# td-kwj-zp2023/webgpu-msm-twisted-edwards

Measured on AMD Instinct MI355X. Metric: MSMs/sec at n=2^20 Twisted-Edwards BLS12 (pipelined throughput = 1000/ms_per_step; single-MSM latency in latency_ms), higher is better.
Workload: dtype u32

## Files before the change

webgpu-msm-twisted-edwards_amd/csrc/kernels.hip.hpp:

```cpp
#pragma once
#include <hip/hip_runtime.h>
#include "curve.hpp"

namespace te {

#define TE_BATCH_MAX 8
struct batch_ptrs { const uint4* p[TE_BATCH_MAX]; };
struct batch_slabs { uint32_t s[TE_BATCH_MAX]; };

struct digits_params {
  uint32_t half[10];
  uint32_t zero_digit;
  uint32_t sc_stride;
  uint32_t n, nst;
  int num_windows;
  int w_first, w_step, nw_local;
  uint32_t half_code, logS, P, CH, chunk_len;
};

struct pnt_slot { uint4 q[8]; };
__device__ __forceinline__ void prep_points_block(uint32_t blk, uint4* __restrict__ lds, const uint4* __restrict__ pts, pnt_slot* __restrict__ recs, uint32_t n) {
  const uint32_t t = threadIdx.x, base = blk * 256u;
  const bool active = t < 256u;
  const uint32_t pieces_in = (n - base < 256u ? n - base : 256u) * 4u;
  const uint4* __restrict__ src = pts + (size_t)base * 4u;
  if (active) {
#pragma unroll
    for (int j = 0; j < 4; j++) {
      const uint32_t g = (uint32_t)j * 256u + t;
      lds[g] = src[g < pieces_in ? g : 0u];
    }
  }
  __syncthreads();
  uint4 a0 = make_uint4(0u, 0u, 0u, 0u), a1 = a0, b0 = a0, b1 = a0;
  if (active) { a0 = lds[4 * t + 0]; a1 = lds[4 * t + 1]; b0 = lds[4 * t + 2]; b1 = lds[4 * t + 3]; }
// ... 519 lines not shown
  __syncthreads();
  const uint32_t c0 = cnt_s[t];
  const size_t gb = (size_t)k * g.B + (size_t)p * g.S + t;
  if (!single) {
    if (c0) atomicAdd(&a.bucket_count[gb], c0);
    wait_own_accesses();
    __syncthreads();
    if (t == 0) pj[2] = (handoff_arrive(&a.part_ticket[k * g.P + p]) + 1u == (cntp + TE_L2_CAP - 1u) / TE_L2_CAP) ? 1u : 0u;
    __syncthreads();
    if (pj[2]) (void)seg_plan_block(p, k, t < g.S ? ld_agent(a.bucket_count + gb) : 0u, g, a.pa, PL, pb, cntp, sbp);
    return;
  }
  if (t < g.S) a.bucket_count[gb] = c0;
  const uint32_t ex = seg_plan_block(p, k, c0, g, a.pa, PL, pb, cntp, sbp);
  if (t < g.S) a.pa.bucket_cursor[gb] = pb + ex + c0;
  off_s[t] = ex;
  __syncthreads();
#pragma unroll
  for (int c = 0; c < 5; c++) {
    uint32_t kv[8], iv[8]; piece_group<PK>(r, c, kv, iv);
    const uint32_t e0 = ((uint32_t)c * 256u + t) * 8u;
#pragma unroll
    for (int e = 0; e < 8; e++) {
      const uint32_t pos = e0 + (uint32_t)e;
      if (pos >= head && pos < total) list[atomicAdd(&off_s[kv[e] & 0x7fffu], 1u)] = iv[e] | ((kv[e] >> 15) << 31);
    }
  }
  __syncthreads();
  uint32_t* out = a.sorted + (size_t)k * g.n + pb;
  for (uint32_t s = t; s < cntp; s += 256u) out[s] = list[s];
}

#define TE_ORDER_REGS 32u
__device__ __forceinline__ void order_scatter_block(uint32_t ob, uint32_t nob, uint32_t* __restrict__ lds, const uint32_t* __restrict__ lenv, uint32_t ids,
                                                    const uint32_t* __restrict__ size_hist, uint32_t* __restrict__ rel_cursor,
                                                    uint32_t* __restrict__ order, uint32_t* __restrict__ num_segments, uint32_t max_len) {
  uint32_t* const h = lds; uint32_t* const base = lds + 1024; uint32_t* const sm = lds + 2048;
  const uint32_t per = (ids + nob - 1) / nob;
  const uint32_t lo = min(ids, ob * per), hi = min(ids, lo + per);
  const bool in_regs = per <= TE_ORDER_REGS * 256u;
  uint32_t lv[TE_ORDER_REGS];
  if (in_regs) {
#pragma unroll
    for (uint32_t j = 0; j < TE_ORDER_REGS; j++) { const uint32_t g = lo + j * 256u + threadIdx.x; lv[j] = g < hi ? lenv[g] : TE_SEG_INVALID; }
  }
  for (uint32_t j = threadIdx.x; j < 1024u; j += 256u) h[j] = 0;
  {
    uint32_t run = 0;
    for (uint32_t c = (1023u - min(max_len, 1023u)) >> 8; c < 4u; c++) {
      const uint32_t s = 1023u - (c * 256u + threadIdx.x);
      uint32_t part[TE_HIST_COPIES];
#pragma unroll
      for (uint32_t r = 0; r < TE_HIST_COPIES; r++) part[r] = size_hist[r * 1024u + s];
      uint32_t cnt_s = 0;
#pragma unroll
      for (uint32_t r = 0; r < TE_HIST_COPIES; r++) cnt_s += part[r];
      uint32_t bt;
      const uint32_t ex = block_excl_scan(cnt_s, sm, bt);
      base[s] = run + ex;
      run += bt;
    }
    if (ob == 0 && threadIdx.x == 0) *num_segments = run;
  }
  __syncthreads();
  if (in_regs) {
#pragma unroll
    for (uint32_t j = 0; j < TE_ORDER_REGS; j++) if (lv[j] != TE_SEG_INVALID) atomicAdd(&h[min(lv[j], 1023u)], 1u);
  } else {
    for (uint32_t g = lo + threadIdx.x; g < hi; g += 256u) { const uint32_t l = lenv[g]; if (l != TE_SEG_INVALID) atomicAdd(&h[min(l, 1023u)], 1u); }
  }
  __syncthreads();
  for (uint32_t j = threadIdx.x; j < 1024u; j += 256u) { base[j] += h[j] ? atomicAdd(&rel_cursor[j], h[j]) : 0u; h[j] = 0; }
  __syncthreads();
  if (in_regs) {
#pragma unroll
    for (uint32_t j = 0; j < TE_ORDER_REGS; j++) {
      if (lv[j] == TE_SEG_INVALID) continue;
      const uint32_t sz = min(lv[j], 1023u);
      order[base[sz] + atomicAdd(&h[sz], 1u)] = lo + j * 256u + threadIdx.x;
    }
  } else {
    for (uint32_t g = lo + threadIdx.x; g < hi; g += 256u) {
      const uint32_t l = lenv[g];
      if (l == TE_SEG_INVALID) continue;
      const uint32_t sz = min(l, 1023u);
      order[base[sz] + atomicAdd(&h[sz], 1u)] = g;
    }
  }
}

#define TE_PLACE_LDS_WORDS (4u * 256u + TE_L2_LIST + TE_L2_LIST / 4u + 2u + 17u)
template <bool PK>
__device__ __forceinline__ void l2_place_piece(uint32_t p, uint32_t k, uint32_t a0, uint32_t b0, uint32_t* __restrict__ lds,
                                               const uint16_t* __restrict__ part_keys, const uint32_t* __restrict__ part_idx,
                                               uint32_t* __restrict__ bucket_cursor, uint32_t* __restrict__ sorted, const sort_geom& g) {
  uint32_t* const cnt_s = lds; uint32_t* const lex_s = lds + 256; uint32_t* const off_s = lds + 512; uint32_t* const gbase_s = lds + 768;
  uint32_t* const list = lds + 1024;
  uint8_t* const list_b = reinterpret_cast<uint8_t*>(list + TE_L2_LIST);
  uint32_t* const sm = list + TE_L2_LIST + TE_L2_LIST / 4u + 2u;
  const uint32_t t = threadIdx.x, len = b0 - a0;
  const uint16_t* keys_row = part_keys + (size_t)k * g.nst; const uint32_t* idx_row = part_idx + (size_t)k * g.nst;
  uint32_t* out = sorted + (size_t)k * g.n;
  cnt_s[t] = 0u;
  __syncthreads();
  piece_regs r; uint32_t head, total;
  load_piece<PK>(keys_row, idx_row, a0, b0, t, true, r, head, total);
#pragma unroll
  for (int c = 0; c < 5; c++) {
    uint32_t kv[8], iv[8]; piece_group<PK>(r, c, kv, iv);
    const uint32_t e0 = ((uint32_t)c * 256u + t) * 8u;
#pragma unroll
    for (int e = 0; e < 8; e++) { const uint32_t pos = e0 + (uint32_t)e; if (pos >= head && pos < total) atomicAdd(&cnt_s[kv[e] & 0x7fffu], 1u); }
  }
  __syncthreads();
  wave0_excl_scan(cnt_s, lex_s, 256u, &sm[16]);
  {
    const uint32_t c0 = cnt_s[t];
    gbase_s[t] = c0 ? atomicAdd(&bucket_cursor[(size_t)k * g.B + (size_t)p * g.S + t], c0) : 0u;
  }
  __syncthreads();
  off_s[t] = lex_s[t];
  gbase_s[t] -= lex_s[t];
  __syncthreads();
#pragma unroll
  for (int c = 0; c < 5; c++) {
    uint32_t kv[8], iv[8]; piece_group<PK>(r, c, kv, iv);
    const uint32_t e0 = ((uint32_t)c * 256u + t) * 8u;
#pragma unroll
    for (int e = 0; e < 8; e++) {
      const uint32_t pos = e0 + (uint32_t)e;
      if (pos >= head && pos < total) {
        const uint32_t b = kv[e] & 0x7fffu;
        const uint32_t slot = atomicAdd(&off_s[b], 1u);
        list[slot] = iv[e] | ((kv[e] >> 15) << 31); list_b[slot] = (uint8_t)b;
      }
    }
  }
  __syncthreads();
  for (uint32_t s = t; s < len; s += 256u) out[gbase_s[list_b[s]] + s] = list[s];
}

struct order_args { const uint32_t* lenv; uint32_t ids; const uint32_t* size_hist; uint32_t* rel_cursor; uint32_t* order; uint32_t* num_segments; uint32_t order_cols, max_len; };
template <bool PK>
__global__ void __launch_bounds__(256, TE_L2_WAVES) k_l2_place_order(const uint16_t* __restrict__ part_keys, const uint32_t* __restrict__ part_idx,
                                                           const uint32_t* __restrict__ part_start, const uint32_t* __restrict__ part_count,
                                                           uint32_t* __restrict__ bucket_cursor, uint32_t* __restrict__ sorted, sort_geom g, order_args oa) {
  __shared__ uint32_t lds[TE_PLACE_LDS_WORDS];
  if (blockIdx.x < oa.order_cols) {
    order_scatter_block(blockIdx.y * oa.order_cols + blockIdx.x, gridDim.y * oa.order_cols, lds, oa.lenv, oa.ids, oa.size_hist, oa.rel_cursor, oa.order, oa.num_segments, oa.max_len);
    return;
  }
  const uint32_t k = gridDim.y - 1u - blockIdx.y;
  const uint32_t px = blockIdx.x - oa.order_cols, extra = gridDim.x - oa.order_cols - g.P, bx = px < extra ? g.P + px : px - extra;
  const uint32_t* pc = part_count + k * g.P;
  uint32_t p, j;
  if (!l2_piece_of_block(bx, pc, g.P, bx < g.P ? 0u : part_count[gridDim.y * g.P + k], lds, lds + 32, p, j)) return;
  const uint32_t cntp = pc[p], pb = part_start[k * g.P + p];
  if (cntp <= TE_L2_CAP) return;
  const uint32_t a0 = pb + j * TE_L2_CAP;
  l2_place_piece<PK>(p, k, a0, min(pb + cntp, a0 + TE_L2_CAP), lds, part_keys, part_idx, bucket_cursor, sorted, g);
}

template <int N> struct geo {
  static constexpr uint32_t PW = 4u * N;
  static constexpr uint32_t PQ = PW / 4u;
  static constexpr uint32_t RW = N == 9 ? 27u : 4u * N;
  static constexpr uint32_t SQ = N == 9 ? 8u : N;
  static constexpr uint32_t LQ = (RW + 3u) / 4u;
};
template <int N> struct rec_slot { uint4 q[geo<N>::SQ]; };
static_assert(sizeof(rec_slot<9>) == sizeof(pnt_slot) && sizeof(rec_slot<14>) == 224, "record slots");

template <int N> __device__ __forceinline__ pnt_t<N> load_pnt(const rec_slot<N>* __restrict__ recs, uint32_t entry) {
  const uint4* q = recs[entry & 0x7fffffffu].q;
  constexpr uint32_t LQ = geo<N>::LQ;
  uint4 u[LQ];
#pragma unroll
  for (uint32_t j = 0; j < LQ; j++) u[j] = q[j];
  uint32_t w[4 * LQ];
#pragma unroll
  for (uint32_t j = 0; j < LQ; j++) { w[4 * j] = u[j].x; w[4 * j + 1] = u[j].y; w[4 * j + 2] = u[j].z; w[4 * j + 3] = u[j].w; }
  pnt_t<N> r;
// ... 45 lines not shown
  const uint32_t* base = recs[entry & 0x7fffffffu].w;
  u4a8 u[10];
#pragma unroll
  for (int j = 0; j < 10; j++) u[j] = reinterpret_cast<const u4a8*>(base)[j];
  const u2a8 t = *reinterpret_cast<const u2a8*>(base + 40);
  uint32_t w[42];
#pragma unroll
  for (int j = 0; j < 10; j++) { w[4 * j] = u[j].v[0]; w[4 * j + 1] = u[j].v[1]; w[4 * j + 2] = u[j].v[2]; w[4 * j + 3] = u[j].v[3]; }
  w[40] = t.v[0]; w[41] = t.v[1];
  pnt_aff377 r;
#pragma unroll
  for (int j = 0; j < 14; j++) { r.hm.v[j] = w[j]; r.hp.v[j] = w[14 + j]; r.dt.v[j] = w[28 + j]; }
  return r;
}
__device__ __forceinline__ void store_pnt_aff377(rec_aff377* dst, const pnt_aff377& r) {
#pragma unroll
  for (int j = 0; j < 14; j++) { dst->w[j] = r.hm.v[j]; dst->w[14 + j] = r.hp.v[j]; dst->w[28 + j] = r.dt.v[j]; }
}
template <int N, int RK> struct rec_kind;
template <int N> struct rec_kind<N, 0> {
  using slot = rec_slot<N>; using pnt = pnt_t<N>;
  static __device__ __forceinline__ pnt load(const slot* __restrict__ recs, uint32_t e) { return load_pnt<N>(recs, e); }
};
template <> struct rec_kind<14, 1> {
  using slot = rec_aff377; using pnt = pnt_aff377;
  static __device__ __forceinline__ pnt load(const slot* __restrict__ recs, uint32_t e) { return load_pnt_aff377(recs, e); }
};

struct __attribute__((aligned(4))) idx4 { uint32_t v[4]; };
#define TE_CLK_SLOTS 64u
#define TE_IDX_STRIP 16u
template <int N, int RK = 0>
__global__ void __attribute__((amdgpu_flat_work_group_size(1, 256), amdgpu_waves_per_eu(N == 9 ? 3 : 2, N == 9 ? 3 : 2))) k_accumulate(const typename rec_kind<N, RK>::slot* __restrict__ recs, const uint32_t* __restrict__ sorted,
                                                    const uint32_t* __restrict__ bucket_start, const uint32_t* __restrict__ bucket_count,
                                                    const uint32_t* __restrict__ seg_base, const uint32_t* __restrict__ seg_bucket,
                                                    const uint32_t* __restrict__ seg_lenv, const uint32_t* __restrict__ order,
                                                    const uint32_t* __restrict__ num_segments, ete_t<N>* __restrict__ buckets,
                                                    ete_t<N>* __restrict__ seg_out, uint32_t n, uint32_t logB, uint32_t seg_len, uint32_t ids, uint32_t onto,
                                                    uint32_t win_per_msm, batch_slabs slabs, unsigned long long* __restrict__ clk) {
  __shared__ __attribute__((aligned(16))) uint32_t idx_strip[256 * TE_IDX_STRIP];
  using RT = rec_kind<N, RK>; using P = typename RT::pnt;
  unsigned long long* const slot = clk ? clk + (blockIdx.x & (TE_CLK_SLOTS - 1u)) : nullptr;
  const unsigned long long t0_wall = clk ? (unsigned long long)wall_clock64() : 0ull, t0_core = clk ? (unsigned long long)clock64() : 0ull;
  if (clk && threadIdx.x == 0) atomicMax(slot, ~t0_wall);
  const uint32_t gid = blockIdx.x * 256u + threadIdx.x;
  if (gid >= (order ? *num_segments : ids)) return;
  const uint32_t sgm = order ? order[gid] : gid;
  const uint32_t g = seg_bucket[sgm];
  if (g == TE_SEG_INVALID) return;
  const uint32_t k = g >> logB;
  recs += (size_t)slabs.s[k / win_per_msm] * n;
  const uint32_t part = sgm - seg_base[g];
  const uint32_t cnt = seg_lenv[sgm];
  const uint32_t* lst = sorted + (size_t)k * n + bucket_start[g] + part * seg_len;
  ete_t<N> acc = (onto && part == 0u) ? load_ete<N>(buckets + g) : ete_identity_t<N>();
  if (cnt) {
    const uint32_t last = cnt - 1u;
    uint32_t j0 = 0;
    uint32_t e = lst[0], e_n = lst[min(1u, last)];
    const uint32_t e_2 = lst[min(2u, last)], e_3 = lst[min(3u, last)];
    P cur = RT::load(recs, e);
    if (!(onto && part == 0u)) {
      const P first = pnt_cneg(cur, (e >> 31) != 0u);
      if (cnt >= 2u) {
        const P second = pnt_cneg(RT::load(recs, e_n), (e_n >> 31) != 0u);
        e = e_2; e_n = e_3;
        cur = RT::load(recs, e);
        acc = ete_from_pair(first, second);
        j0 = 2;
      } else {
        acc = ete_from_pnt(first);
        j0 = 1;
      }
    }
    uint32_t* const strip = idx_strip + threadIdx.x * TE_IDX_STRIP;
    auto refill = [&](uint32_t pos) {
      const idx4* src = reinterpret_cast<const idx4*>(lst + pos);
      idx4* dst = reinterpret_cast<idx4*>(strip);
#pragma unroll
      for (uint32_t h = 0; h < TE_IDX_STRIP / 4u; h += 2u) {
        const idx4 v0 = src[h], v1 = src[h + 1u];
        dst[h] = v0; dst[h + 1u] = v1;
      }
    };
    if (((j0 + 2u) & (TE_IDX_STRIP - 1u)) != 0u) refill((j0 + 2u) & ~(TE_IDX_STRIP - 1u));
    P rec_b;
    uint32_t j = j0;
    for (; j + 2u < cnt; j += 2u) {
      const uint32_t pn = j + 2u;
      if ((pn & (TE_IDX_STRIP - 1u)) == 0u) refill(pn);
      const uint2 e_nn = *reinterpret_cast<const uint2*>(strip + (pn & (TE_IDX_STRIP - 1u)));
      rec_b = RT::load(recs, e_n);
      acc = ete_madd(acc, pnt_cneg(cur, (e >> 31) != 0u));
      __builtin_amdgcn_sched_barrier(0);
      cur = RT::load(recs, e_nn.x);
      acc = ete_madd(acc, pnt_cneg(rec_b, (e_n >> 31) != 0u));
      e = e_nn.x; e_n = e_nn.y;
    }
    if (j < cnt) {
      const bool two = j + 1u < cnt;
      rec_b = RT::load(recs, two ? e_n : e);
      acc = ete_madd(acc, pnt_cneg(cur, (e >> 31) != 0u));
      if (two) acc = ete_madd(acc, pnt_cneg(rec_b, (e_n >> 31) != 0u));
    }
  }
  const bool whole = bucket_count[g] <= seg_len;
  store_ete<N>(whole ? buckets + g : seg_out + sgm, acc);
  if (clk && (uint32_t)__lane_id() == (uint32_t)__ffsll((long long)__ballot(1)) - 1u) {
    const unsigned long long t1_wall = (unsigned long long)wall_clock64(), t1_core = (unsigned long long)clock64();
    atomicMax(slot + TE_CLK_SLOTS, t1_wall);
    atomicAdd(slot + 2u * TE_CLK_SLOTS, t1_core - t0_core); atomicAdd(slot + 3u * TE_CLK_SLOTS, t1_wall - t0_wall);
  }
}

template <int N> struct sum_job_t {
  const ete_t<N>* in; ete_t<N>* out;
  uint32_t n_out;
  uint32_t K, inner;
  uint32_t in_per_window, out_per_window;
};
template <int N> struct sum_jobs_t { sum_job_t<N> j[4]; };
template <int N> __device__ __forceinline__ ete_t<N> pair_swap(const ete_t<N>& a) {
  ete_t<N> r;
#pragma unroll
  for (int i = 0; i < N; i++) {
    r.x.v[i] = (uint32_t)__builtin_amdgcn_mov_dpp((int)a.x.v[i], 0xb1, 0xf, 0xf, true);
    r.y.v[i] = (uint32_t)__builtin_amdgcn_mov_dpp((int)a.y.v[i], 0xb1, 0xf, 0xf, true);
    r.z.v[i] = (uint32_t)__builtin_amdgcn_mov_dpp((int)a.z.v[i], 0xb1, 0xf, 0xf, true);
    r.t.v[i] = (uint32_t)__builtin_amdgcn_mov_dpp((int)a.t.v[i], 0xb1, 0xf, 0xf, true);
  }
  return r;
}
template <int N, bool PAIR>
__global__ void __launch_bounds__(256, N == 9 ? 2 : 1) k_sum_groups(sum_jobs_t<N> js, uint32_t nw) {
  const sum_job_t<N>& j = js.j[blockIdx.y];
  constexpr uint32_t TPO = PAIR ? 2u : 1u;
  const uint32_t total = j.n_out * nw * TPO, Kt = j.K / TPO;
  for (uint32_t gt = blockIdx.x * 256u + threadIdx.x; gt < total; gt += gridDim.x * 256u) {
    const uint32_t g = gt / TPO, half = gt % TPO;
    const uint32_t k = g / j.n_out, o = g - k * j.n_out;
// ... 511 lines not shown
```

webgpu-msm-twisted-edwards_amd/csrc/te_msm.hip:

```cpp
#include <hip/hip_runtime.h>
#include <stdint.h>
#include <stdio.h>
#include <stdlib.h>
#include <string.h>
#include <string>
#include <vector>
#include <deque>
#include <algorithm>
#include <functional>
#include <chrono>
#include <thread>
#include <mutex>
#include <condition_variable>
#include <memory>
#include <optional>
#include <type_traits>
#if defined(__x86_64__)
#include <immintrin.h>
#endif

#include "../../include/te_msm.h"
#include "host_tail.hpp"
#include "synth.hpp"
#include "kernels.hip.hpp"
// ... 24 lines not shown
constexpr size_t TE_MAX_ROW_BYTES = TE377_TAIL_ROW_BYTES;

struct plan_t {
  int curve = 0;
  int c = 0, W = 0, nw = 0;
  int nw1 = 0, batch = 1;
  int w_first = 0, w_step = 1;
  uint32_t B = 0, logB = 0;
  int signed_digits = 1;
  uint32_t dw[4] = {0, 0, 0, 0};
  uint32_t CH = 0, chunk_len = 0, nst = 0;
  uint32_t seg_len = 64;
  uint32_t S = 0, logS = 0, P = 0;
  uint32_t packed = 0;
  int rec_kind = 0;
  int fb_rb = 0, fb_c = 0, fb_W = 0;
};

template <typename T> struct dev_buf {
  T* p = nullptr; size_t cap = 0;
  operator T*() const { return p; }
  void release() { if (p) (void)hipFree(p); p = nullptr; cap = 0; }
};

struct workset_t {
  hipStream_t stream = nullptr, copy_stream = nullptr;
  int hw_queue_class = -1;
  hipEvent_t ev_copy = nullptr, ev_start = nullptr;
  dev_buf<uint8_t> d_recs;
  dev_buf<uint16_t> d_digits, d_part_keys;
  dev_buf<uint32_t> d_part_start, d_part_count, d_part_idx, d_seg_part_base;
  dev_buf<uint32_t> d_bucket_start, d_bucket_cursor, d_sorted;
  dev_buf<uint32_t> d_seg_base, d_seg_bucket, d_seg_lenv, d_order;
  dev_buf<uint32_t> d_split_list, d_chunk_list;
  dev_buf<uint8_t> d_seg_out, d_buckets, d_red[4];
  dev_buf<uint32_t> d_zero; size_t zero_words = 0;
  size_t zero_clean_words = 0;
  uint32_t *d_err = nullptr, *d_num_seg = nullptr, *d_size_hist = nullptr, *d_size_cursor = nullptr, *d_counts1 = nullptr, *d_bucket_count = nullptr;
  uint32_t* d_part_ticket = nullptr;
  uint8_t* d_partials = nullptr;
  uint32_t* h_err = nullptr;
  uint8_t* h_partials = nullptr;
  uint32_t* h_err_dev = nullptr;
  bool rows_on_host = false;
  hipEvent_t ev_done = nullptr;
  hipEvent_t ev_result = nullptr;
  hipEvent_t ev[ST_COUNT + 1] = {};
  plan_t plan; uint64_t n = 0; bool used = false;
  te_sched::slot_t slot;
  std::string job_err;
  int prof_level = 0;
  hipStream_t last_stream = nullptr;
  dev_buf<uint8_t> d_in_points, d_in_scalars;
  std::vector<hipEvent_t> piece_events;
  uint8_t* h_ring = nullptr; std::vector<hipEvent_t> ring_ev; size_t ring_next = 0;
  uint64_t idle_calls = 0;
  dev_buf<uint32_t> d_fb_remap;
  uint32_t* d_fb_fill = nullptr;
  const void* fb_scalars = nullptr; uint64_t fb_n = 0;
  int slab = -1;
  bool slab_run = false;
  const uint8_t* recs_last = nullptr;
  te_bases* bound = nullptr;
  int pt_rc = 0; int64_t pt_index = -1; int pt_reason = 0;
  dev_buf<uint8_t> d_batch_rows;
  dev_buf<uint32_t> d_in_idx;
  template <typename WS, typename F> static void each_buffer(WS& ws, F&& f) {
    f(ws.d_recs); f(ws.d_digits); f(ws.d_part_keys); f(ws.d_part_start); f(ws.d_part_count); f(ws.d_part_idx); f(ws.d_seg_part_base);
    f(ws.d_bucket_start); f(ws.d_bucket_cursor); f(ws.d_sorted); f(ws.d_seg_base); f(ws.d_seg_bucket); f(ws.d_seg_lenv); f(ws.d_order);
    f(ws.d_split_list); f(ws.d_chunk_list); f(ws.d_seg_out); f(ws.d_buckets); for (auto& b : ws.d_red) f(b);
    f(ws.d_zero); f(ws.d_in_points); f(ws.d_in_scalars); f(ws.d_fb_remap); f(ws.d_batch_rows); f(ws.d_in_idx);
  }
};
constexpr int TE_MAX_WINDOWS = 64;
constexpr size_t Z_KEEP = 4;
constexpr size_t Z_ENTRIES = 2;
constexpr size_t Z_CLOCK = 8;
static_assert(Z_KEEP + 4 <= Z_CLOCK && Z_ENTRIES % 2 == 0 && Z_ENTRIES + 2 <= Z_KEEP, "flag words");
constexpr size_t Z_ROWS = Z_CLOCK + 4 * 2 * TE_CLK_SLOTS, Z_HIST = Z_ROWS + (size_t)TE_MAX_WINDOWS * TE_MAX_ROW_BYTES / 4, Z_CURSOR = Z_HIST + 1024 * TE_HIST_COPIES, Z_END = Z_CURSOR + 1024;

struct gpu_t {
  int device = 0;
  int w_first = 0, w_step = 1;
  workset_t ws[TE_MSM_WORKSETS];
  int last_ws = 0;
  int wall_clock_khz = 0;
  int in_flight = 0;
  bool queues_probed = false;
  struct rec_slab_t { const void* src = nullptr; uint64_t n = 0; int curve = 0; uint8_t* d = nullptr; size_t cap = 0; int users = 0;
                      uint32_t pending = 0; hipEvent_t ev[TE_MSM_WORKSETS] = {};
                      int run_users = 0; bool converted = false; hipEvent_t conv_ev = nullptr; };
  std::vector<rec_slab_t> slabs;
  std::unique_ptr<std::mutex> scalar_link{new std::mutex};
  std::unique_ptr<std::mutex> chk_mu{new std::mutex};
  hipStream_t chk_stream = nullptr; dev_buf<uint8_t> chk_pts;
  unsigned long long *chk_word = nullptr, *chk_host = nullptr;
  bool streams_exported = false;
  bool streams_final = false;
  uint8_t* h_batch_rows = nullptr; size_t h_batch_cap = 0;
};

}
// ... 144 lines not shown
}

struct seq_sizes {
  size_t wb, smax;
  size_t chunk_cap(size_t slack = 0) const { return wb + (smax + slack) / TE_GIANT_RUN + 2; }
};
inline seq_sizes sizes_for(const plan_t& p, uint64_t n) {
  const size_t wb = (size_t)p.nw * p.B;
  return {wb, wb + (size_t)p.nw * (size_t)(n / (uint64_t)p.seg_len)};
}

int ensure_buffers(te_ctx* ctx, gpu_t& d, workset_t& ws, uint64_t n, const plan_t& p, bool need_recs = true) {
  HIP_TRY(ctx, hipSetDevice(d.device));
  const seq_sizes sz = sizes_for(p, n);
  const size_t nd = (size_t)p.nw * p.nst + 64, wb = sz.wb, ab = sizes_of(p.curve).acc;
  int rc = 0;
  if (need_recs && (rc = make_room(ctx, ws.d_recs, (size_t)n * sizes_of(p.curve).rec * (size_t)p.batch))) return rc;
  if ((rc = make_room(ctx, ws.d_digits, nd))) return rc;
  if ((rc = make_room(ctx, ws.d_sorted, nd))) return rc;
  {
    const size_t c1 = (size_t)p.nw * p.CH * p.P;
    ws.zero_words = Z_END + c1 + wb + (size_t)p.nw * p.P + 64;
    { const uint32_t* before = ws.d_zero; if ((rc = make_room(ctx, ws.d_zero, ws.zero_words))) return rc; if (ws.d_zero != before) ws.zero_clean_words = 0; }
    ws.d_err = ws.d_zero; ws.d_num_seg = ws.d_zero + Z_KEEP; ws.d_size_hist = ws.d_zero + Z_HIST; ws.d_size_cursor = ws.d_zero + Z_CURSOR;
    ws.d_partials = reinterpret_cast<uint8_t*>(ws.d_zero + Z_ROWS);
    ws.d_counts1 = ws.d_zero + Z_END; ws.d_bucket_count = ws.d_counts1 + c1; ws.d_part_ticket = ws.d_bucket_count + wb;
    ws.d_fb_fill = ws.d_part_ticket + (size_t)p.nw * p.P;
  }
  if (p.fb_rb && (rc = make_room(ctx, ws.d_fb_remap, nd))) return rc;
  if ((rc = make_room(ctx, ws.d_bucket_start, wb))) return rc;
  if ((rc = make_room(ctx, ws.d_bucket_cursor, wb))) return rc;
  if ((rc = make_room(ctx, ws.d_seg_part_base, (size_t)p.nw * p.P))) return rc;
  const size_t smax = sz.smax + 16;
  if ((rc = make_room(ctx, ws.d_order, smax))) return rc;
  if ((rc = make_room(ctx, ws.d_seg_bucket, smax))) return rc;
  if ((rc = make_room(ctx, ws.d_seg_lenv, smax))) return rc;
  if ((rc = make_room(ctx, ws.d_seg_out, smax * ab))) return rc;
  if ((rc = make_room(ctx, ws.d_seg_base, wb + 1))) return rc;
  if ((rc = make_room(ctx, ws.d_split_list, wb + 1))) return rc;
  if ((rc = make_room(ctx, ws.d_chunk_list, 2 * sz.chunk_cap(16)))) return rc;
  if ((rc = make_room(ctx, ws.d_part_start, (size_t)p.nw * p.P))) return rc;
  if ((rc = make_room(ctx, ws.d_buckets, wb * ab))) return rc;
  if ((rc = make_room(ctx, ws.d_part_count, (size_t)p.nw * p.P + (size_t)p.nw))) return rc;
  if ((rc = make_room(ctx, ws.d_part_keys, p.packed ? 8 : nd))) return rc;
  if ((rc = make_room(ctx, ws.d_part_idx, nd))) return rc;
  for (int k = 0; k < 4; k++) if ((rc = make_room(ctx, ws.d_red[k], (wb / (k % 2 ? 4 : 2) + 1) * ab))) return rc;
  return 0;
}

template <int LO, int HI, typename F> void with_window_bits(int c, F&& f) {
  if constexpr (LO < HI) { if (c != LO) return with_window_bits<LO + 1, HI>(c, f); }
  f(std::integral_constant<int, LO>{});
}

template <int C> void launch_digits(const te::batch_ptrs& sc, int batch, uint16_t* dg, const te::digits_params& prm, uint32_t* err, uint32_t* counts1, hipStream_t s) {
  hipLaunchKernelGGL(te::k_digits<C>, dim3((prm.nst + TE_DIG_BLOCK - 1u) / TE_DIG_BLOCK, batch), dim3(TE_DIG_THREADS), 0, s, sc, dg, prm, err, counts1);
}
static_assert(TE_BATCH_MAX == TE_MSM_MAX_BATCH, "batch tables");
template <int C> void launch_digits_ragged(const void* sc, const te::ragged_tab& tab, int batch, uint16_t* dg, const te::digits_params& prm, uint32_t* err, uint32_t* counts1, hipStream_t s) {
  hipLaunchKernelGGL(te::k_digits_ragged<C>, dim3((prm.nst + TE_DIG_BLOCK - 1u) / TE_DIG_BLOCK, batch), dim3(TE_DIG_THREADS), 0, s, static_cast<const uint4*>(sc), tab, dg, prm, err, counts1);
}
static_assert(TE_RAGGED_MAX == TE_BATCH_SEQ_MAX && TE_BATCH_SEQ_MAX == TE_MSM_BATCH_SEQ_MAX, "ragged tables");

struct msm_launch {
  te_ctx* ctx; workset_t& ws; plan_t p;
  const void* d_points = nullptr; const void* d_scalars = nullptr; uint64_t n = 0;
  void* d_partials_out = nullptr;
// ... 95 lines not shown
          const uint32_t per_row = (n32 + 511u) / 512u;
          hipLaunchKernelGGL(te::k_part_scatter_prep377, dim3(sblocks + rows * per_row), dim3(512), 0, stream, sa, sblocks, tab, row_slab,
                             reinterpret_cast<te::rec_slot<14>*>(recs_out()), n32, per_row, rows * per_row);
        } else {
          const uint32_t per_row = (n32 + 255u) / 256u;
          hipLaunchKernelGGL(te::k_part_scatter_prep, dim3(sblocks + rows * per_row), dim3(512), 0, stream, sa, sblocks, tab, row_slab,
                             reinterpret_cast<te::pnt_slot*>(recs_out()), n32, per_row, rows * per_row);
        }
      } else if (idx) {
        hipLaunchKernelGGL(te::k_part_scatter_indexed, dim3(p.CH, p.nw), dim3(512), 0, stream, sa, te::index_args{idx, idx_count, idx_pos, ws.d_err});
      } else {
        hipLaunchKernelGGL(te::k_part_scatter, dim3(p.CH, p.nw), dim3(512), 0, stream, sa);
      }
    }
    mark(ST_BSORT);
    if (p.nw > 0) {
      const uint32_t l2_blocks = p.P + n32 / TE_L2_CAP + 1u;
      te::l2_args la;
      la.part_keys = ws.d_part_keys; la.part_idx = ws.d_part_idx; la.part_start = ws.d_part_start; la.part_count = ws.d_part_count;
      la.bucket_count = ws.d_bucket_count; la.sorted = ws.d_sorted; la.part_ticket = ws.d_part_ticket; la.g = sg;
      la.pa.part_start = ws.d_part_start; la.pa.part_count = ws.d_part_count; la.pa.seg_part_base = ws.d_seg_part_base;
      la.pa.bucket_start = ws.d_bucket_start; la.pa.bucket_cursor = ws.d_bucket_cursor; la.pa.seg_base = ws.d_seg_base; la.pa.seg_bucket = ws.d_seg_bucket;
      la.pa.seg_lenv = ws.d_seg_lenv; la.pa.size_hist = ws.d_size_hist; la.pa.split_list = ws.d_split_list; la.pa.split_count = ws.d_num_seg + 1;
      la.pa.chunk_list = ws.d_chunk_list; la.pa.seg_len = p.seg_len; la.pa.cap_w = cap_w; la.pa.chunk_cap = chunk_cap();
      if (p.packed) hipLaunchKernelGGL(te::k_l2_local<true>, dim3(l2_blocks, p.nw), dim3(256), 0, stream, la);
      else hipLaunchKernelGGL(te::k_l2_local<false>, dim3(l2_blocks, p.nw), dim3(256), 0, stream, la);
      te::order_args oa;
      oa.lenv = ws.d_seg_lenv; oa.ids = smax(); oa.size_hist = ws.d_size_hist; oa.rel_cursor = ws.d_size_cursor; oa.order = ws.d_order; oa.num_segments = ws.d_num_seg;
      {
        const uint32_t by_regs = (smax() + TE_ORDER_REGS * 256u * (uint32_t)p.nw - 1u) / (TE_ORDER_REGS * 256u * (uint32_t)p.nw);
        oa.order_cols = std::min(64u, std::max(by_regs, (uint32_t)std::max(1, 128 / p.nw)));
      }
      oa.max_len = std::min(p.seg_len, 1023u);
      if (p.packed)
        hipLaunchKernelGGL(te::k_l2_place_order<true>, dim3(oa.order_cols + l2_blocks, p.nw), dim3(256), 0, stream, ws.d_part_keys, ws.d_part_idx, ws.d_part_start,
                           ws.d_part_count, ws.d_bucket_cursor, ws.d_sorted, sg, oa);
      else
        hipLaunchKernelGGL(te::k_l2_place_order<false>, dim3(oa.order_cols + l2_blocks, p.nw), dim3(256), 0, stream, ws.d_part_keys, ws.d_part_idx, ws.d_part_start,
                           ws.d_part_count, ws.d_bucket_cursor, ws.d_sorted, sg, oa);
    }
    mark(ST_ORDER);
    return 0;
  }

  bool bls() const { return p.curve == TE_MSM_CURVE_BLS12_377_G1; }

  template <int N, int RK> int accumulate_t() {
    mark(ST_ACCUM);
    if (p.nw > 0) {
      const uint32_t n32 = this->n32(), smax = this->smax();
      const uint32_t* order = ctx->opt_sort ? ws.d_order : nullptr;
      using slot_t = typename te::rec_kind<N, RK>::slot;
      hipLaunchKernelGGL((te::k_accumulate<N, RK>), dim3((smax + 255) / 256), dim3(256), 0, stream, reinterpret_cast<const slot_t*>(bound ? bound : recs_out()), ws.d_sorted,
                         ws.d_bucket_start, ws.d_bucket_count, ws.d_seg_base, ws.d_seg_bucket, ws.d_seg_lenv, order, ws.d_num_seg,
                         reinterpret_cast<te::ete_t<N>*>(ws.d_buckets.p), reinterpret_cast<te::ete_t<N>*>(ws.d_seg_out.p), n32, p.logB, p.seg_len, smax, onto ? 1u : 0u,
                         ragged ? (uint32_t)p.nw : (uint32_t)p.nw1, ragged ? te::batch_slabs{} : slabs(),
                         prof ? reinterpret_cast<unsigned long long*>(ws.d_zero + Z_CLOCK) : nullptr);
    }
    return 0;
  }
  int accumulate() { return bls() ? (p.rec_kind == 1 ? accumulate_t<14, 1>() : accumulate_t<14, 0>()) : accumulate_t<9, 0>(); }

  template <int N> int combine_t() {
    if (p.nw <= 0) return 0;
    using E = te::ete_t<N>;
    hipLaunchKernelGGL(te::k_seg_combine_all<N>, dim3(256 + 1024), dim3(256), 0, stream, ws.d_split_list, ws.d_num_seg + 1, ws.d_chunk_list,
                       ws.d_bucket_count, ws.d_seg_base, reinterpret_cast<E*>(ws.d_seg_out.p), reinterpret_cast<E*>(ws.d_buckets.p), p.seg_len, chunk_cap(), 256u,
                       ws.d_bucket_start, ws.d_bucket_cursor);
    return 0;
  }
  int combine() { return bls() ? combine_t<14>() : combine_t<9>(); }

  template <int N> int reduce_t() {
    if (p.nw > 0) {
      using E = te::ete_t<N>;
      const uint32_t w0 = p.dw[0], w1 = p.dw[1], w2 = p.dw[2], w3 = p.dw[3];
      const uint32_t L = 1u << (w0 + w1), H = 1u << (w2 + w3);
      struct chain_t { const E* cur; uint32_t n, r; E* buf[2]; int pp; };
      E* const bk = reinterpret_cast<E*>(ws.d_buckets.p);
      chain_t ch[2] = {{bk, p.B, L, {reinterpret_cast<E*>(ws.d_red[0].p), reinterpret_cast<E*>(ws.d_red[1].p)}, 0},
                       {bk, p.B, H, {reinterpret_cast<E*>(ws.d_red[2].p), reinterpret_cast<E*>(ws.d_red[3].p)}, 0}};
      for (;;) {
        te::sum_jobs_t<N> js; memset(&js, 0, sizeof js);
        uint32_t most = 0; int nj = 0;
        for (int i = 0; i < 2; i++) {
          chain_t& c = ch[i];
          if (c.r <= 4u) continue;
          const uint32_t K = (c.r % 8u == 0) ? 8u : (c.r % 4u == 0) ? 4u : 2u;
// ... 2580 lines not shown
  if (device_index < 0 || (size_t)device_index >= ctx->devs.size() || first > total || count > total - first) return set_err(ctx, TE_MSM_EINVAL, "bad arguments");
  if (record_bytes) *record_bytes = (int)bases->rec_bytes;
  uint64_t bytes = count * bases->rec_bytes;
  if (bytes > cap) bytes = cap;
  if (!bytes) return 0;
  HIP_TRY(ctx, hipSetDevice(ctx->devs[(size_t)device_index].device));
  HIP_TRY(ctx, hipMemcpy(dst, bases->recs[(size_t)device_index] + first * bases->rec_bytes, bytes, hipMemcpyDeviceToHost));
  return (int64_t)bytes;
}

int64_t te_msm_debug_read(te_ctx* ctx, const char* stage, void* dst, uint64_t cap) {
  device_guard restore_callers_device;
  if (!ctx || !stage || !dst) return TE_MSM_EINVAL;
  drain_workers(ctx);
  gpu_t& d = ctx->devs[0];
  workset_t& ws = d.ws[d.last_ws];
  if (!ws.used) return set_err(ctx, TE_MSM_ESTATE, "no run yet");
  const plan_t& p = ws.plan; const uint64_t n = ws.n;
  const void* src = nullptr; uint64_t bytes = 0;
  if (ws.zero_clean_words && (!strcmp(stage, "bucket_count") || !strcmp(stage, "num_segments") || !strcmp(stage, "partials")))
    return set_err(ctx, TE_MSM_ESTATE, "this stage lives in the block that is cleared behind an MSM's read-back: set option prezero = 0 before the run to keep it");
  if (!strcmp(stage, "records")) {
    if (!ws.recs_last) return set_err(ctx, TE_MSM_ESTATE, "the last run gathered from a bound point set: the work set holds no records of its own");
    src = ws.recs_last; bytes = n * sizes_of(p.curve).rec;
  }
  else if (!strcmp(stage, "digits")) { src = ws.d_digits; bytes = (uint64_t)p.nw * p.nst * 2; }
  else if (!strcmp(stage, "bucket_count")) { src = ws.d_bucket_count; bytes = (uint64_t)p.nw * p.B * 4; }
  else if (!strcmp(stage, "bucket_start")) { src = ws.d_bucket_start; bytes = (uint64_t)p.nw * p.B * 4; }
  else if (!strcmp(stage, "sorted")) { src = ws.d_sorted; bytes = (uint64_t)p.nw * n * 4; }
  else if (!strcmp(stage, "num_segments")) { src = ws.d_num_seg; bytes = 4; }
  else if (!strcmp(stage, "seg_bucket")) { src = ws.d_seg_bucket; bytes = ((uint64_t)p.nw * p.B + (uint64_t)p.nw * (n / p.seg_len)) * 4; }
  else if (!strcmp(stage, "seg_len")) { src = ws.d_seg_lenv; bytes = ((uint64_t)p.nw * p.B + (uint64_t)p.nw * (n / p.seg_len)) * 4; }
  else if (!strcmp(stage, "order")) { src = ws.d_order; bytes = ((uint64_t)p.nw * p.B + (uint64_t)p.nw * (n / p.seg_len)) * 4; }
  else if (!strcmp(stage, "part_start")) { src = ws.d_part_start; bytes = (uint64_t)p.nw * p.P * 4; }
  else if (!strcmp(stage, "part_count")) { src = ws.d_part_count; bytes = (uint64_t)p.nw * p.P * 4; }
  else if (!strcmp(stage, "part_keys") && !p.packed) { src = ws.d_part_keys; bytes = (uint64_t)p.nw * p.nst * 2; }
  else if (!strcmp(stage, "part_idx") && !p.packed) { src = ws.d_part_idx; bytes = (uint64_t)p.nw * p.nst * 4; }
  else if (!strcmp(stage, "part_keys") || !strcmp(stage, "part_idx")) {
    const bool want_keys = stage[5] == 'k';
    const uint64_t words = (uint64_t)p.nw * p.nst;
    std::vector<uint32_t> pk(words);
    HIP_TRY(ctx, hipSetDevice(d.device));
    HIP_TRY(ctx, hipDeviceSynchronize());
    HIP_TRY(ctx, hipMemcpy(pk.data(), ws.d_part_idx, words * 4, hipMemcpyDeviceToHost));
    uint64_t out_bytes = words * (want_keys ? 2 : 4);
    if (out_bytes > cap) out_bytes = cap;
    if (want_keys) { uint16_t* o = static_cast<uint16_t*>(dst); for (uint64_t i = 0; i < out_bytes / 2; i++) o[i] = (uint16_t)(((pk[i] >> 23) & 0xffu) | ((pk[i] >> 31) << 15)); }
    else { uint32_t* o = static_cast<uint32_t*>(dst); for (uint64_t i = 0; i < out_bytes / 4; i++) o[i] = pk[i] & 0x7fffffu; }
    return (int64_t)out_bytes;
  }
  else if (!strcmp(stage, "buckets")) { src = ws.d_buckets; bytes = (uint64_t)p.nw * p.B * sizes_of(p.curve).acc; }
  else if (!strcmp(stage, "partials")) { src = ws.d_partials; bytes = (uint64_t)p.W * sizes_of(p.curve).row; }
  else return set_err(ctx, TE_MSM_EINVAL, "unknown stage");
  if (bytes > cap) bytes = cap;
  HIP_TRY(ctx, hipSetDevice(d.device));
  HIP_TRY(ctx, hipDeviceSynchronize());
  HIP_TRY(ctx, hipMemcpy(dst, src, bytes, hipMemcpyDeviceToHost));
  return (int64_t)bytes;
}

}
```

Baseline: 1148.

## Precompute packed segment descriptors in order scatter for accumulate kernel

The order-scatter stage now writes a 16-byte descriptor per segment, either in sorted order or indexed by id. It packs bucket, list position, count, id and first/whole flags. The accumulate kernel reads this one coalesced uint4 instead of chasing order, seg_bucket, seg_base, bucket_start, bucket_count and seg_lenv through dependent gathers. This removes the latency of the indirect-load chain at the start of accumulate. In exchange, order scatter does extra gathers and writes, and a new buffer adds memory traffic.

Result: no change. 1142 (-0.6%).

```diff
diff --git a/webgpu-msm-twisted-edwards_amd/csrc/kernels.hip.hpp b/webgpu-msm-twisted-edwards_amd/csrc/kernels.hip.hpp
--- a/webgpu-msm-twisted-edwards_amd/csrc/kernels.hip.hpp
+++ b/webgpu-msm-twisted-edwards_amd/csrc/kernels.hip.hpp
@@ -1,6 +1,7 @@
 #pragma once
 #include <hip/hip_runtime.h>
 #include "curve.hpp"
+#include "seg_desc.hpp"
 
 namespace te {
 
@@ -586,9 +587,15 @@
 }
 
 #define TE_ORDER_REGS 32u
+struct desc_src { const uint32_t *seg_bucket, *seg_base, *bucket_start, *bucket_count; uint4* desc; uint32_t seg_len, by_id; };
+__device__ __forceinline__ void desc_store(uint4* __restrict__ dst, const te_segdesc::words& d) { *dst = make_uint4(d.w[0], d.w[1], d.w[2], d.w[3]); }
+__device__ __forceinline__ te_segdesc::words desc_of(uint32_t id, uint32_t len, uint32_t g, uint32_t sbase, uint32_t bstart, uint32_t bcount, uint32_t seg_len) {
+  const uint32_t part = id - sbase;
+  return te_segdesc::pack(g, bstart + part * seg_len, len, id, part == 0u, bcount <= seg_len);
+}
 __device__ __forceinline__ void order_scatter_block(uint32_t ob, uint32_t nob, uint32_t* __restrict__ lds, const uint32_t* __restrict__ lenv, uint32_t ids,
                                                     const uint32_t* __restrict__ size_hist, uint32_t* __restrict__ rel_cursor,
-                                                    uint32_t* __restrict__ order, uint32_t* __restrict__ num_segments, uint32_t max_len) {
+                                                    uint32_t* __restrict__ order, uint32_t* __restrict__ num_segments, uint32_t max_len, const desc_src& ds) {
   uint32_t* const h = lds; uint32_t* const base = lds + 1024; uint32_t* const sm = lds + 2048;
   const uint32_t per = (ids + nob - 1) / nob;
   const uint32_t lo = min(ids, ob * per), hi = min(ids, lo + per);
@@ -628,17 +635,34 @@
   __syncthreads();
   if (in_regs) {
 #pragma unroll
-    for (uint32_t j = 0; j < TE_ORDER_REGS; j++) {
-      if (lv[j] == TE_SEG_INVALID) continue;
-      const uint32_t sz = min(lv[j], 1023u);
-      order[base[sz] + atomicAdd(&h[sz], 1u)] = lo + j * 256u + threadIdx.x;
+    for (uint32_t j0 = 0; j0 < TE_ORDER_REGS; j0 += 8u) {
+      uint32_t gb[8], sb[8], bs[8], bc[8];
+#pragma unroll
+      for (uint32_t e = 0; e < 8u; e++) gb[e] = lv[j0 + e] != TE_SEG_INVALID ? ds.seg_bucket[lo + (j0 + e) * 256u + threadIdx.x] : 0u;
+#pragma unroll
+      for (uint32_t e = 0; e < 8u; e++) {
+        const bool v = lv[j0 + e] != TE_SEG_INVALID;
+        sb[e] = v ? ds.seg_base[gb[e]] : 0u; bs[e] = v ? ds.bucket_start[gb[e]] : 0u; bc[e] = v ? ds.bucket_count[gb[e]] : 0u;
+      }
+#pragma unroll
+      for (uint32_t e = 0; e < 8u; e++) {
+        const uint32_t id = lo + (j0 + e) * 256u + threadIdx.x, l = lv[j0 + e];
+        if (l == TE_SEG_INVALID) { if (ds.by_id && id < hi) desc_store(ds.desc + id, te_segdesc::invalid()); continue; }
+        const uint32_t sz = min(l, 1023u);
+        const uint32_t pos = base[sz] + atomicAdd(&h[sz], 1u);
+        order[pos] = id;
+        desc_store(ds.desc + (ds.by_id ? id : pos), desc_of(id, l, gb[e], sb[e], bs[e], bc[e], ds.seg_len));
+      }
     }
   } else {
-    for (uint32_t g = lo + threadIdx.x; g < hi; g += 256u) {
-      const uint32_t l = lenv[g];
-      if (l == TE_SEG_INVALID) continue;
+    for (uint32_t id = lo + threadIdx.x; id < hi; id += 256u) {
+      const uint32_t l = lenv[id];
+      if (l == TE_SEG_INVALID) { if (ds.by_id) desc_store(ds.desc + id, te_segdesc::invalid()); continue; }
       const uint32_t sz = min(l, 1023u);
-      order[base[sz] + atomicAdd(&h[sz], 1u)] = g;
+      const uint32_t pos = base[sz] + atomicAdd(&h[sz], 1u);
+      order[pos] = id;
+      const uint32_t g = ds.seg_bucket[id];
+      desc_store(ds.desc + (ds.by_id ? id : pos), desc_of(id, l, g, ds.seg_base[g], ds.bucket_start[g], ds.bucket_count[g], ds.seg_len));
     }
   }
 }
@@ -694,14 +718,14 @@
   for (uint32_t s = t; s < len; s += 256u) out[gbase_s[list_b[s]] + s] = list[s];
 }
 
-struct order_args { const uint32_t* lenv; uint32_t ids; const uint32_t* size_hist; uint32_t* rel_cursor; uint32_t* order; uint32_t* num_segments; uint32_t order_cols, max_len; };
+struct order_args { const uint32_t* lenv; uint32_t ids; const uint32_t* size_hist; uint32_t* rel_cursor; uint32_t* order; uint32_t* num_segments; uint32_t order_cols, max_len; desc_src ds; };
 template <bool PK>
 __global__ void __launch_bounds__(256, TE_L2_WAVES) k_l2_place_order(const uint16_t* __restrict__ part_keys, const uint32_t* __restrict__ part_idx,
                                                            const uint32_t* __restrict__ part_start, const uint32_t* __restrict__ part_count,
                                                            uint32_t* __restrict__ bucket_cursor, uint32_t* __restrict__ sorted, sort_geom g, order_args oa) {
   __shared__ uint32_t lds[TE_PLACE_LDS_WORDS];
   if (blockIdx.x < oa.order_cols) {
-    order_scatter_block(blockIdx.y * oa.order_cols + blockIdx.x, gridDim.y * oa.order_cols, lds, oa.lenv, oa.ids, oa.size_hist, oa.rel_cursor, oa.order, oa.num_segments, oa.max_len);
+    order_scatter_block(blockIdx.y * oa.order_cols + blockIdx.x, gridDim.y * oa.order_cols, lds, oa.lenv, oa.ids, oa.size_hist, oa.rel_cursor, oa.order, oa.num_segments, oa.max_len, oa.ds);
     return;
   }
   const uint32_t k = gridDim.y - 1u - blockIdx.y;
@@ -813,11 +837,9 @@
 #define TE_IDX_STRIP 16u
 template <int N, int RK = 0>
 __global__ void __attribute__((amdgpu_flat_work_group_size(1, 256), amdgpu_waves_per_eu(N == 9 ? 3 : 2, N == 9 ? 3 : 2))) k_accumulate(const typename rec_kind<N, RK>::slot* __restrict__ recs, const uint32_t* __restrict__ sorted,
-                                                    const uint32_t* __restrict__ bucket_start, const uint32_t* __restrict__ bucket_count,
-                                                    const uint32_t* __restrict__ seg_base, const uint32_t* __restrict__ seg_bucket,
-                                                    const uint32_t* __restrict__ seg_lenv, const uint32_t* __restrict__ order,
+                                                    const uint4* __restrict__ desc,
                                                     const uint32_t* __restrict__ num_segments, ete_t<N>* __restrict__ buckets,
-                                                    ete_t<N>* __restrict__ seg_out, uint32_t n, uint32_t logB, uint32_t seg_len, uint32_t ids, uint32_t onto,
+                                                    ete_t<N>* __restrict__ seg_out, uint32_t n, uint32_t logB, uint32_t ids, uint32_t onto,
                                                     uint32_t win_per_msm, batch_slabs slabs, unsigned long long* __restrict__ clk) {
   __shared__ __attribute__((aligned(16))) uint32_t idx_strip[256 * TE_IDX_STRIP];
   using RT = rec_kind<N, RK>; using P = typename RT::pnt;
@@ -825,15 +847,16 @@
   const unsigned long long t0_wall = clk ? (unsigned long long)wall_clock64() : 0ull, t0_core = clk ? (unsigned long long)clock64() : 0ull;
   if (clk && threadIdx.x == 0) atomicMax(slot, ~t0_wall);
   const uint32_t gid = blockIdx.x * 256u + threadIdx.x;
-  if (gid >= (order ? *num_segments : ids)) return;
-  const uint32_t sgm = order ? order[gid] : gid;
-  const uint32_t g = seg_bucket[sgm];
-  if (g == TE_SEG_INVALID) return;
+  if (gid >= (num_segments ? *num_segments : ids)) return;
+  const uint4 dq = desc[gid];
+  const te_segdesc::words dw{{dq.x, dq.y, dq.z, dq.w}};
+  if (!te_segdesc::is_valid(dw)) return;
+  const te_segdesc::fields sd = te_segdesc::unpack(dw);
+  const uint32_t g = sd.g, sgm = sd.id, cnt = sd.cnt;
   const uint32_t k = g >> logB;
   recs += (size_t)slabs.s[k / win_per_msm] * n;
-  const uint32_t part = sgm - seg_base[g];
-  const uint32_t cnt = seg_lenv[sgm];
-  const uint32_t* lst = sorted + (size_t)k * n + bucket_start[g] + part * seg_len;
+  const uint32_t part = sd.first ? 0u : 1u;
+  const uint32_t* lst = sorted + (size_t)k * n + sd.pos;
   ete_t<N> acc = (onto && part == 0u) ? load_ete<N>(buckets + g) : ete_identity_t<N>();
   if (cnt) {
     const uint32_t last = cnt - 1u;
@@ -885,8 +908,7 @@
       if (two) acc = ete_madd(acc, pnt_cneg(rec_b, (e_n >> 31) != 0u));
     }
   }
-  const bool whole = bucket_count[g] <= seg_len;
-  store_ete<N>(whole ? buckets + g : seg_out + sgm, acc);
+  store_ete<N>(sd.whole ? buckets + g : seg_out + sgm, acc);
   if (clk && (uint32_t)__lane_id() == (uint32_t)__ffsll((long long)__ballot(1)) - 1u) {
     const unsigned long long t1_wall = (unsigned long long)wall_clock64(), t1_core = (unsigned long long)clock64();
     atomicMax(slot + TE_CLK_SLOTS, t1_wall);
diff --git a/webgpu-msm-twisted-edwards_amd/csrc/seg_desc.hpp b/webgpu-msm-twisted-edwards_amd/csrc/seg_desc.hpp
--- /dev/null
+++ b/webgpu-msm-twisted-edwards_amd/csrc/seg_desc.hpp
@@ -0,0 +1,40 @@
+#pragma once
+
+#include <cstdint>
+
+#if defined(__HIPCC__) || defined(__CUDACC__)
+#define TE_SD_FN __host__ __device__ __forceinline__
+#else
+#define TE_SD_FN inline
+#endif
+
+namespace te_segdesc {
+
+constexpr uint32_t kInvalid = 0xffffffffu;
+constexpr uint32_t kBucketBits = 30u;
+constexpr uint32_t kBucketMask = (1u << kBucketBits) - 1u;
+constexpr uint32_t kFirstBit = 1u << 30, kWholeBit = 1u << 31;
+constexpr uint64_t kMaxBuckets = (1ull << kBucketBits) - 1u;
+constexpr uint64_t kMaxEntries = 1ull << 32;
+constexpr uint64_t kMaxIds = 0xffffffffull;
+
+struct words { uint32_t w[4]; };
+struct fields {
+  uint32_t g, pos, cnt, id;
+  bool first;
+  bool whole;
+};
+
+TE_SD_FN bool fits(uint64_t buckets, uint64_t n, uint64_t ids) { return buckets <= kMaxBuckets && n < kMaxEntries && ids <= kMaxIds; }
+TE_SD_FN bool packable(uint64_t g, uint64_t pos, uint64_t cnt, uint64_t id) { return g < kMaxBuckets && pos < kMaxEntries && cnt < kMaxEntries && id < kMaxIds; }
+
+TE_SD_FN words pack(uint32_t g, uint32_t pos, uint32_t cnt, uint32_t id, bool first, bool whole) {
+  return words{{g | (first ? kFirstBit : 0u) | (whole ? kWholeBit : 0u), pos, cnt, id}};
+}
+TE_SD_FN words invalid() { return words{{kInvalid, 0u, 0u, kInvalid}}; }
+TE_SD_FN bool is_valid(const words& d) { return d.w[0] != kInvalid; }
+TE_SD_FN fields unpack(const words& d) {
+  return fields{d.w[0] & kBucketMask, d.w[1], d.w[2], d.w[3], (d.w[0] & kFirstBit) != 0u, (d.w[0] & kWholeBit) != 0u};
+}
+
+}
diff --git a/webgpu-msm-twisted-edwards_amd/csrc/te_msm.hip b/webgpu-msm-twisted-edwards_amd/csrc/te_msm.hip
--- a/webgpu-msm-twisted-edwards_amd/csrc/te_msm.hip
+++ b/webgpu-msm-twisted-edwards_amd/csrc/te_msm.hip
@@ -80,6 +80,7 @@
   dev_buf<uint32_t> d_part_start, d_part_count, d_part_idx, d_seg_part_base;
   dev_buf<uint32_t> d_bucket_start, d_bucket_cursor, d_sorted;
   dev_buf<uint32_t> d_seg_base, d_seg_bucket, d_seg_lenv, d_order;
+  dev_buf<uint4> d_seg_desc;
   dev_buf<uint32_t> d_split_list, d_chunk_list;
   dev_buf<uint8_t> d_seg_out, d_buckets, d_red[4];
   dev_buf<uint32_t> d_zero; size_t zero_words = 0;
@@ -115,7 +116,7 @@
   dev_buf<uint32_t> d_in_idx;
   template <typename WS, typename F> static void each_buffer(WS& ws, F&& f) {
     f(ws.d_recs); f(ws.d_digits); f(ws.d_part_keys); f(ws.d_part_start); f(ws.d_part_count); f(ws.d_part_idx); f(ws.d_seg_part_base);
-    f(ws.d_bucket_start); f(ws.d_bucket_cursor); f(ws.d_sorted); f(ws.d_seg_base); f(ws.d_seg_bucket); f(ws.d_seg_lenv); f(ws.d_order);
+    f(ws.d_bucket_start); f(ws.d_bucket_cursor); f(ws.d_sorted); f(ws.d_seg_base); f(ws.d_seg_bucket); f(ws.d_seg_lenv); f(ws.d_order); f(ws.d_seg_desc);
     f(ws.d_split_list); f(ws.d_chunk_list); f(ws.d_seg_out); f(ws.d_buckets); for (auto& b : ws.d_red) f(b);
     f(ws.d_zero); f(ws.d_in_points); f(ws.d_in_scalars); f(ws.d_fb_remap); f(ws.d_batch_rows); f(ws.d_in_idx);
   }
@@ -326,7 +327,9 @@
   if ((rc = make_room(ctx, ws.d_bucket_cursor, wb))) return rc;
   if ((rc = make_room(ctx, ws.d_seg_part_base, (size_t)p.nw * p.P))) return rc;
   const size_t smax = sz.smax + 16;
+  if (!te_segdesc::fits(wb, n, smax)) return set_err(ctx, TE_MSM_EINVAL, "plan beyond the segment descriptor's fields: buckets < 2^30 - 1, n < 2^32, segment ids < 2^32 - 1");
   if ((rc = make_room(ctx, ws.d_order, smax))) return rc;
+  if ((rc = make_room(ctx, ws.d_seg_desc, smax))) return rc;
   if ((rc = make_room(ctx, ws.d_seg_bucket, smax))) return rc;
   if ((rc = make_room(ctx, ws.d_seg_lenv, smax))) return rc;
   if ((rc = make_room(ctx, ws.d_seg_out, smax * ab))) return rc;
@@ -488,6 +491,8 @@
         oa.order_cols = std::min(64u, std::max(by_regs, (uint32_t)std::max(1, 128 / p.nw)));
       }
       oa.max_len = std::min(p.seg_len, 1023u);
+      oa.ds.seg_bucket = ws.d_seg_bucket; oa.ds.seg_base = ws.d_seg_base; oa.ds.bucket_start = ws.d_bucket_start; oa.ds.bucket_count = ws.d_bucket_count;
+      oa.ds.desc = ws.d_seg_desc; oa.ds.seg_len = p.seg_len; oa.ds.by_id = ctx->opt_sort ? 0u : 1u;
       if (p.packed)
         hipLaunchKernelGGL(te::k_l2_place_order<true>, dim3(oa.order_cols + l2_blocks, p.nw), dim3(256), 0, stream, ws.d_part_keys, ws.d_part_idx, ws.d_part_start,
                            ws.d_part_count, ws.d_bucket_cursor, ws.d_sorted, sg, oa);
@@ -505,11 +510,10 @@
     mark(ST_ACCUM);
     if (p.nw > 0) {
       const uint32_t n32 = this->n32(), smax = this->smax();
-      const uint32_t* order = ctx->opt_sort ? ws.d_order : nullptr;
       using slot_t = typename te::rec_kind<N, RK>::slot;
       hipLaunchKernelGGL((te::k_accumulate<N, RK>), dim3((smax + 255) / 256), dim3(256), 0, stream, reinterpret_cast<const slot_t*>(bound ? bound : recs_out()), ws.d_sorted,
-                         ws.d_bucket_start, ws.d_bucket_count, ws.d_seg_base, ws.d_seg_bucket, ws.d_seg_lenv, order, ws.d_num_seg,
-                         reinterpret_cast<te::ete_t<N>*>(ws.d_buckets.p), reinterpret_cast<te::ete_t<N>*>(ws.d_seg_out.p), n32, p.logB, p.seg_len, smax, onto ? 1u : 0u,
+                         ws.d_seg_desc.p, ctx->opt_sort ? ws.d_num_seg : nullptr,
+                         reinterpret_cast<te::ete_t<N>*>(ws.d_buckets.p), reinterpret_cast<te::ete_t<N>*>(ws.d_seg_out.p), n32, p.logB, smax, onto ? 1u : 0u,
                          ragged ? (uint32_t)p.nw : (uint32_t)p.nw1, ragged ? te::batch_slabs{} : slabs(),
                          prof ? reinterpret_cast<unsigned long long*>(ws.d_zero + Z_CLOCK) : nullptr);
     }
@@ -3156,6 +3160,8 @@
   else if (!strcmp(stage, "seg_bucket")) { src = ws.d_seg_bucket; bytes = ((uint64_t)p.nw * p.B + (uint64_t)p.nw * (n / p.seg_len)) * 4; }
   else if (!strcmp(stage, "seg_len")) { src = ws.d_seg_lenv; bytes = ((uint64_t)p.nw * p.B + (uint64_t)p.nw * (n / p.seg_len)) * 4; }
   else if (!strcmp(stage, "order")) { src = ws.d_order; bytes = ((uint64_t)p.nw * p.B + (uint64_t)p.nw * (n / p.seg_len)) * 4; }
+  else if (!strcmp(stage, "seg_desc")) { src = ws.d_seg_desc; bytes = ((uint64_t)p.nw * p.B + (uint64_t)p.nw * (n / p.seg_len)) * 16; }
+  else if (!strcmp(stage, "seg_base")) { src = ws.d_seg_base; bytes = (uint64_t)p.nw * p.B * 4; }
   else if (!strcmp(stage, "part_start")) { src = ws.d_part_start; bytes = (uint64_t)p.nw * p.P * 4; }
   else if (!strcmp(stage, "part_count")) { src = ws.d_part_count; bytes = (uint64_t)p.nw * p.P * 4; }
   else if (!strcmp(stage, "part_keys") && !p.packed) { src = ws.d_part_keys; bytes = (uint64_t)p.nw * p.nst * 2; }
```
